# PeterFWS/Structure-PLP-SLAM

Hardware: NVIDIA H100
Metric: frames_per_sec_extract_match_poseopt (higher is better)
Workload: dtype u8/f64

## Files before the change

structure-plp-slam_b200/csrc/orb.cu:

```cuda
#include "common.cuh"
#include <cuda.h>
#include <stdlib.h>
#include "brief_pattern.inc"

namespace plp {

namespace {

constexpr int kMaxLevels = 16;
constexpr int kPatchRadius = 19;
constexpr int kHalfPatch = 15;
constexpr int kCellSize = 64;
constexpr int kOverlap = 6;
constexpr int kCellCap = 1024;

struct LevelInfo {
    int w, h, pitch;
    size_t offset;
    size_t blur_offset;
    int cells_x, cells_y;
    int cell_base;
    int num_cells;
    int budget;
    int slot_base;
// ... 802 lines not shown
    const int g = gx * gy;
    int cur = 0, cur_n = 0, len = 0;
    {
        int *cnts = S.scan;
        for (int i = tid; i < g; i += kQtThreads) cnts[i] = 0;
        __syncthreads();
        for (int i = tid; i < n; i += kQtThreads) {
            const uint32_t c = A.cand[i];
            const unsigned ix = (unsigned)((float)cand_x(c) / dx), iy = (unsigned)((float)cand_y(c) / dy);
            int node = (int)(ix + iy * gx);
            node = min(node, g - 1);
            cls[i] = 0;
            A.owner[0][i] = (unsigned short)node;
            atomicAdd(&cnts[node], 1);
        }
        __syncthreads();
        if (tid == 0) {
            int off = 0, pos = 0;
            for (int i = 0; i < g; ++i) {
                const int c = cnts[i];
                S.newpos[i] = off;
                if (c > 0) {
                    const int ix = i % gx, iy = i / gx;
                    short4 r;
                    r.x = (short)(int)(dx * ix);
                    r.y = (short)(int)(dy * iy);
                    r.z = (short)(int)(dx * (ix + 1));
                    r.w = (short)(int)(dy * (iy + 1));
                    S.rect[0][pos] = r;
                    S.start[0][pos] = (unsigned short)off;
                    S.cnt[0][pos] = (unsigned short)c;
                    S.leaf[0][pos] = (c == 1);
                    S.tot[i] = (unsigned short)pos;
                    ++pos;
                }
                off += c;
            }
            S.misc[0] = pos;
        }
        __syncthreads();
        len = S.misc[0];
        for (int node = 0; node < g; ++node) {
            if (cnts[node] == 0) continue;
            const int per = (n + kQtThreads - 1) / kQtThreads;
            const int i0 = min(n, tid * per), i1 = min(n, i0 + per);
            int c = 0;
            for (int i = i0; i < i1; ++i) c += (A.owner[0][i] == node);
            int tot;
            int run = block_exclusive_scan(c, S.warp_tmp, &tot);
            const int base = S.newpos[node];
            const unsigned short lp = S.tot[node];
            for (int i = i0; i < i1; ++i)
                if (A.owner[0][i] == node) {
                    A.perm[1][base + run] = (unsigned short)i;
                    A.owner[1][base + run] = lp;
                    ++run;
                }
            __syncthreads();
        }
        cur = 1;
    }
    const int budget = LV.budget;
    int pool_len = 0, pool_cur = 0;
    bool filled = false;
    unsigned short *proc_list = S.pool_sorted;

    while (true) {
        const int prev = len;
        for (int p = tid; p < len; p += kQtThreads) S.sel[p] = S.leaf[cur_n][p] ? 0 : 1;
        __syncthreads();
        for (int p = tid; p < len; p += kQtThreads) S.scan[p] = S.sel[p];
        __syncthreads();
        const int num_proc = block_scan_array(S.scan, len, S.warp_tmp);
        for (int p = tid; p < len; p += kQtThreads)
            if (S.sel[p]) proc_list[S.scan[p]] = (unsigned short)p;
        __syncthreads();
        segmented_class_scan(A, cur, n, QtNodes{S.rect[cur_n], S.start[cur_n], S.cnt[cur_n], S.leaf[cur_n]}, S.sel,
                             rank, cls, S.tot, S.carry_tail, S.carry_head);
        len = apply_division(S, A, cur, n, cur_n, len, num_proc, proc_list, rank, cls, &pool_len, pool_cur);
        if (budget <= len || len == prev) {
            filled = true;
            break;
        }
        if (budget < len + pool_len) break;
    }
    while (!filled) {
        const int prev = len;
        const unsigned short *pool = S.pool[pool_cur];
        for (int p = tid; p < len; p += kQtThreads) S.sel[p] = 0;
        __syncthreads();
        for (int k = tid; k < pool_len; k += kQtThreads) S.sel[pool[k]] = 1;
        __syncthreads();
        segmented_class_scan(A, cur, n, QtNodes{S.rect[cur_n], S.start[cur_n], S.cnt[cur_n], S.leaf[cur_n]}, S.sel,
                             rank, cls, S.tot, S.carry_tail, S.carry_head);
        for (int k = tid; k < pool_len; k += kQtThreads) {
            const int ck = S.cnt[cur_n][pool[k]];
            int r = 0;
            for (int j = 0; j < pool_len; ++j) {
                const int cj = S.cnt[cur_n][pool[j]];
                r += (cj > ck) || (cj == ck && j > k);
            }
            proc_list[r] = pool[k];
        }
        __syncthreads();
        for (int k = tid; k < pool_len; k += kQtThreads) {
            const unsigned short *t = S.tot + proc_list[k] * 4;
            S.scan[k] = (t[0] > 0) + (t[1] > 0) + (t[2] > 0) + (t[3] > 0) - 1;
        }
        if (tid == 0) {
            S.misc[1] = pool_len;
            S.misc[2] = 0;
        }
        __syncthreads();
        block_scan_array(S.scan, pool_len, S.warp_tmp);
        for (int k = tid; k < pool_len; k += kQtThreads) {
            const unsigned short *t = S.tot + proc_list[k] * 4;
            const int inc = (t[0] > 0) + (t[1] > 0) + (t[2] > 0) + (t[3] > 0) - 1;
            if (prev + S.scan[k] + inc >= budget) {
                atomicMin(&S.misc[1], k + 1);
                S.misc[2] = 1;
            }
        }
        __syncthreads();
        const int num_proc = S.misc[1];
        const bool reached = S.misc[2] != 0;
        __syncthreads();
        for (int k = num_proc + tid; k < pool_len; k += kQtThreads) S.sel[proc_list[k]] = 0;
        __syncthreads();
        len = apply_division(S, A, cur, n, cur_n, len, num_proc, proc_list, rank, cls, &pool_len, pool_cur ^ 1);
        pool_cur ^= 1;
        if (reached) filled = true;
        if (filled || budget <= len || len == prev) break;
    }

    const int n_out = min(len, LV.slot_cap);
    if (len > LV.slot_cap && tid == 0) P.status[b] = 3;
    for (int p = tid; p < n_out; p += kQtThreads) {
        const int st = S.start[cur_n][p], c = S.cnt[cur_n][p];
        uint32_t best = A.cand[A.perm[cur][st]];
        for (int k = 1; k < c; ++k) {
            const uint32_t v = A.cand[A.perm[cur][st + k]];
            if (cand_score(v) > cand_score(best)) best = v;
        }
        LevelKp kp;
        kp.x = (short)(cand_x(best) + kPatchRadius);
        kp.y = (short)(cand_y(best) + kPatchRadius);
        kp.response = cand_score(best);
        out[p] = kp;
    }
    if (tid == 0) *lvl_cnt = n_out;
}

constexpr int kDescWarps = 4;
constexpr int kBlurDim = 39, kBlurPitch = 44;

__device__ __forceinline__ int reflect101(int p, int len) {
    if (p < 0) p = -p;
    if (p >= len) p = 2 * (len - 1) - p;
    return p;
}

__device__ __forceinline__ float fast_atan2_deg(float y, float x) {
    const float scale = (float)(180.0 / 3.14159265358979323846);
    const float p1 = 0.9997878412794807f * scale, p3 = -0.3258083974640975f * scale,
                p5 = 0.1555786518463281f * scale, p7 = -0.04432655554792128f * scale;
    const float ax = fabsf(x), ay = fabsf(y);
    float a, c, c2;
    if (ax >= ay) {
        c = __fdiv_rn(ay, ax + (float)2.2204460492503131e-16);
        c2 = c * c;
        a = (((p7 * c2 + p5) * c2 + p3) * c2 + p1) * c;
    } else {
        c = __fdiv_rn(ax, ay + (float)2.2204460492503131e-16);
        c2 = c * c;
        a = 90.f - (((p7 * c2 + p5) * c2 + p3) * c2 + p1) * c;
    }
    if (x < 0) a = 180.f - a;
    if (y < 0) a = 360.f - a;
    return a;
}

__device__ __forceinline__ float poly_cos(float v) {
    const float c1 = 0.99940307f, c2 = -0.49558072f, c3 = 0.03679168f;
    const float v2 = v * v;
    return c1 + v2 * (c2 + c3 * v2);
}
__device__ __forceinline__ float util_cos(float v) {
    const float PI = 3.14159265358979f, PI_2 = PI / 2.0f, TWO_PI = 2.0f * PI, INV_TWO_PI = 1.0f / TWO_PI,
                THREE_PI_2 = 3.0f * PI_2;
    v = v - (float)cv_floor((double)(v * INV_TWO_PI)) * TWO_PI;
    v = (0.0f < v) ? v : -v;
    if (v < PI_2) return poly_cos(v);
    if (v < PI) return -poly_cos(PI - v);
    if (v < THREE_PI_2) return -poly_cos(v - PI);
    return poly_cos(TWO_PI - v);
}
__device__ __forceinline__ float util_sin(float v) {
    const float PI_2 = 3.14159265358979f / 2.0f;
    return util_cos(PI_2 - v);
}


__device__ __forceinline__ void blur_row4(const uint32_t *w, uint32_t h[4]) {
    const uint32_t A = w[0], B = w[1], C = w[2];
    const uint32_t kW1 = 0x38302212u, kW2 = 0x00122230u;
    h[0] = __dp4a(__funnelshift_r(A, B, 8), kW1, __dp4a(__funnelshift_r(B, C, 8), kW2, 0u));
    h[1] = __dp4a(__funnelshift_r(A, B, 16), kW1, __dp4a(__funnelshift_r(B, C, 16), kW2, 0u));
    h[2] = __dp4a(__funnelshift_r(A, B, 24), kW1, __dp4a(__funnelshift_r(B, C, 24), kW2, 0u));
    h[3] = __dp4a(B, kW1, __dp4a(C, kW2, 0u));
}
__device__ __forceinline__ void blur_h_pass(const uint8_t *box, uint32_t *h2) {
    const uint32_t *src32 = reinterpret_cast<const uint32_t *>(box);
    for (int i = threadIdx.x; i < (kBoxH / 2) * (kBtW / 4); i += blockDim.x) {
        const int rp = i / (kBtW / 4), j = i % (kBtW / 4);
        const uint32_t *w = src32 + 2 * rp * (kBoxW / 4) + j + (kBoxX - 4) / 4;
        uint32_t e[4], o[4];
        blur_row4(w, e);
        blur_row4(w + kBoxW / 4, o);
        *reinterpret_cast<uint4 *>(h2 + rp * kBtW + 4 * j) =
            make_uint4(__byte_perm(e[0], o[0], 0x5410), __byte_perm(e[1], o[1], 0x5410), __byte_perm(e[2], o[2], 0x5410),
                       __byte_perm(e[3], o[3], 0x5410));
    }
}

constexpr int kBlurThreads = 256;
static_assert((kBtH / 2) * (kBtW / 4) == kBlurThreads, "one vertical-pass job per thread");
__device__ __forceinline__ void blur_v_pass(const uint32_t *h2, uint8_t *dst, int dpitch, int x0, int y0, int W, int H) {
    const int q = threadIdx.x / (kBtW / 4), px = (threadIdx.x % (kBtW / 4)) * 4;
    const int y = y0 + 2 * q;
    if (y >= H || x0 + px >= W) return;
    uint32_t r[4][4];
#pragma unroll
    for (int k = 0; k < 4; ++k) {
        const uint4 v = *reinterpret_cast<const uint4 *>(h2 + (q + k) * kBtW + px);
        r[k][0] = v.x;
        r[k][1] = v.y;
        r[k][2] = v.z;
        r[k][3] = v.w;
    }
    auto row = [&](uint32_t k0, uint32_t k1, uint32_t k2, uint32_t k3) -> uint32_t {
        uint32_t a[4];
#pragma unroll
        for (int c = 0; c < 4; ++c)
            a[c] = __dp2a_lo(r[0][c], k0, __dp2a_lo(r[1][c], k1, __dp2a_lo(r[2][c], k2, __dp2a_lo(r[3][c], k3, 32768u))));
        return __byte_perm(__byte_perm(a[0], a[1], 0x0062), __byte_perm(a[2], a[3], 0x0062), 0x5410);
    };
    uint8_t *d = dst + (size_t)y * dpitch + x0 + px;
    *reinterpret_cast<uint32_t *>(d) = row(0x2212u, 0x3830u, 0x2230u, 0x0012u);
    if (y + 1 < H) *reinterpret_cast<uint32_t *>(d + dpitch) = row(0x1200u, 0x3022u, 0x3038u, 0x1222u);
}

__global__ void __launch_bounds__(kBlurThreads) blur_tiles_kernel(OrbDev P) {
    __shared__ __align__(16) uint8_t s_src[kBoxH * kBoxW];
    __shared__ __align__(16) uint32_t s_h2[(kBoxH / 2) * kBtW];
    const int b = blockIdx.y, tid = threadIdx.x;
    const BlurTile t = P.blur_tiles[blockIdx.x];
    const int l = t.level, W = P.lv[l].w, H = P.lv[l].h;
    const uint8_t *img = level_ptr(P, b, l);
    const int pitch = level_pitch(P, l);
    constexpr int kCols = kBtW + 8;
    for (int i = tid; i < kBoxH * kCols; i += kBlurThreads) {
        const int py = i / kCols, px = i - py * kCols;
        const int gy = reflect101(min(t.y0 - 3 + py, H + 2), H);
        const int gx = reflect101(min(max(t.x0 - 4 + px, -3), W + 2), W);
        s_src[py * kBoxW + kBoxX - 4 + px] = img[(size_t)gy * pitch + gx];
    }
    __syncthreads();
    blur_h_pass(s_src, s_h2);
    __syncthreads();
    blur_v_pass(s_h2, P.blur + (size_t)b * P.blur_frame_bytes + P.lv[l].blur_offset, P.lv[l].pitch, t.x0, t.y0, W, H);
}

__device__ void blur_reflect_box(uint8_t *box, int bx0, int by0, int W, int H) {
    for (int i = threadIdx.x; i < kBoxH * 6; i += blockDim.x) {
        const int py = i / 6, k = i - py * 6;
        const int gx = k < 3 ? k - 3 : W + (k - 3), gy = by0 + py;
        const int px = gx - bx0;
        if (gy < 0 || gy >= H || px < 0 || px >= kBoxW) continue;
        box[py * kBoxW + px] = box[py * kBoxW + (reflect101(gx, W) - bx0)];
    }
    __syncthreads();
    for (int i = threadIdx.x; i < 6 * kBoxW; i += blockDim.x) {
        const int k = i / kBoxW, px = i - k * kBoxW;
        const int gy = k < 3 ? k - 3 : H + (k - 3);
        const int py = gy - by0;
        if (py < 0 || py >= kBoxH) continue;
        box[py * kBoxW + px] = box[(reflect101(gy, H) - by0) * kBoxW + px];
    }
    __syncthreads();
}

constexpr int kBlurRun = 4;
template <bool kMapsInGlobal>
__global__ void __launch_bounds__(kBlurThreads) blur_tiles_tma_kernel(const __grid_constant__ BlurMaps M, const CUtensorMap *gmaps,
                                                                      OrbDev P, int run) {
    __shared__ __align__(128) uint8_t s_src[2][kBoxStage];
    __shared__ __align__(16) uint32_t s_h2[(kBoxH / 2) * kBtW];
    __shared__ __align__(8) unsigned long long s_bar[2];
    const int b = blockIdx.y, tid = threadIdx.x;
    const int first = blockIdx.x * run, n = min(run, P.num_blur_tiles - first);
    if (tid == 0) {
        mbar_init(smem_u32(&s_bar[0]));
        mbar_init(smem_u32(&s_bar[1]));
        asm volatile("fence.mbarrier_init.release.cluster;" ::: "memory");
    }
    __syncthreads();
    auto issue = [&](int i) {
        const BlurTile t = P.blur_tiles[first + i];
        const uint32_t bar = smem_u32(&s_bar[i & 1]);
        mbar_expect_tx(bar, kBoxH * kBoxW);
        tma_box_load(smem_u32(s_src[i & 1]), level_map<kMapsInGlobal>(M, gmaps, t.level), t.x0 - kBoxX, t.y0 - 3, b, bar);
    };
    if (tid == 0) issue(0);
    for (int i = 0; i < n; ++i) {
        __syncthreads();
        if (tid == 0 && i + 1 < n) {
            asm volatile("fence.proxy.async.shared::cta;" ::: "memory");
            issue(i + 1);
        }
        const BlurTile t = P.blur_tiles[first + i];
        const int l = t.level, W = P.lv[l].w, H = P.lv[l].h;
        const int bx0 = t.x0 - kBoxX, by0 = t.y0 - 3;
        uint8_t *box = s_src[i & 1];
        if (!mbar_wait(smem_u32(&s_bar[i & 1]), (i >> 1) & 1)) P.status[b] = 3;
        if (t.x0 < 3 || by0 < 0 || t.x0 + kBtW + 3 > W || by0 + kBoxH > H) blur_reflect_box(box, bx0, by0, W, H);
        blur_h_pass(box, s_h2);
        __syncthreads();
        blur_v_pass(s_h2, P.blur + (size_t)b * P.blur_frame_bytes + P.lv[l].blur_offset, P.lv[l].pitch, t.x0, t.y0, W, H);
    }
}

__global__ void __launch_bounds__(kDescWarps * 32) describe_kernel(OrbDev P, plp_keypoint *__restrict__ kp_out,
                                                                    uint8_t *__restrict__ desc_out,
                                                                    int32_t *__restrict__ n_out) {
    __shared__ __align__(16) uint8_t s_win[kDescWarps][kBlurDim * kBlurPitch];
    const int b = blockIdx.y, warp = threadIdx.x >> 5, lane = threadIdx.x & 31;
    __shared__ int s_cum[kMaxLevels + 1];
    __shared__ const uint8_t *s_img[kMaxLevels], *s_blur[kMaxLevels];
    __shared__ int s_pitch[kMaxLevels], s_bpitch[kMaxLevels], s_slot[kMaxLevels];
    __shared__ float s_scale[kMaxLevels], s_size[kMaxLevels];
    if (threadIdx.x == 0) {
        const int *lvl_cnt = P.lvl_cnt + (size_t)b * P.num_levels;
        int acc = 0;
        for (int l = 0; l < P.num_levels; ++l) {
            s_cum[l] = acc;
            acc += lvl_cnt[l];
        }
        for (int l = P.num_levels; l <= kMaxLevels; ++l) s_cum[l] = acc;
    }
    if (threadIdx.x < P.num_levels) {
        const int l = threadIdx.x;
        s_img[l] = level_ptr(P, b, l);
        s_pitch[l] = level_pitch(P, l);
        s_blur[l] = P.blur + (size_t)b * P.blur_frame_bytes + P.lv[l].blur_offset;
        s_bpitch[l] = P.lv[l].pitch;
        s_slot[l] = P.lv[l].slot_base;
        s_scale[l] = P.lv[l].scale_factor;
        s_size[l] = P.lv[l].size;
    }
    __syncthreads();
    const int total = min(s_cum[kMaxLevels], P.out_cap);
    if (blockIdx.x == 0 && threadIdx.x == 0) n_out[b] = total;
    const LevelKp *frame_kp = P.lvl_kp + (size_t)b * P.total_slots;
    for (int out_pos = blockIdx.x * kDescWarps + warp; out_pos < total; out_pos += gridDim.x * kDescWarps) {
    int l = 0;
    while (out_pos >= s_cum[l + 1]) ++l;
    const LevelKp kp = frame_kp[s_slot[l] + out_pos - s_cum[l]];
    const uint8_t *img = s_img[l];
    const int pitch = s_pitch[l];
    const int cx = kp.x, cy = kp.y;

    int m10 = 0, m01 = 0;
    {
        constexpr int kUmax[16] = {15, 15, 15, 15, 14, 14, 14, 13, 13, 12, 11, 10, 9, 8, 6, 3};
        const int u = lane - kHalfPatch;
        const int au = u < 0 ? -u : u;
        const uint8_t *c0 = img + (size_t)cy * pitch + cx + u;
#pragma unroll
        for (int v = -kHalfPatch; v <= kHalfPatch; ++v) {
            const int d = kUmax[v < 0 ? -v : v];
            if (lane < 31 && au <= d) {
                const int val = __ldg(c0 + v * pitch);
                m10 += u * val;
                m01 += v * val;
            }
        }
#pragma unroll
        for (int o = 16; o > 0; o >>= 1) {
            m10 += __shfl_xor_sync(0xffffffffu, m10, o);
            m01 += __shfl_xor_sync(0xffffffffu, m01, o);
        }
    }
    const float angle = fast_atan2_deg((float)m01, (float)m10);

    const float ang_rad = (float)((double)angle * 3.14159265358979323846 / 180.0);
    const float ca = util_cos(ang_rad), sa = util_sin(ang_rad);
    const int bpitch = s_bpitch[l];
    const int wx0 = cx - 19, woff = wx0 & 3, nwords = (woff + kBlurDim + 3) >> 2;
    const uint8_t *bsrc = s_blur[l] + (size_t)(cy - 19) * bpitch + (wx0 - woff);
    uint8_t *win = s_win[warp];
    __syncwarp();
    {
        const int half = lane >> 4, j = lane & 15;
        if (j < nwords) {
#pragma unroll 5
            for (int r = half; r < kBlurDim; r += 2)
                *reinterpret_cast<uint32_t *>(win + r * kBlurPitch + 4 * j) =
                    __ldg(reinterpret_cast<const uint32_t *>(bsrc + (size_t)r * bpitch) + j);
        }
    }
    __syncwarp();
    const uint8_t *center = win + 19 * kBlurPitch + 19 + woff;
    int val = 0;
    const uint2 px1 = __ldg(reinterpret_cast<const uint2 *>(kBriefX1) + lane), py1 = __ldg(reinterpret_cast<const uint2 *>(kBriefY1) + lane);
    const uint2 px2 = __ldg(reinterpret_cast<const uint2 *>(kBriefX2) + lane), py2 = __ldg(reinterpret_cast<const uint2 *>(kBriefY2) + lane);
#pragma unroll
    for (int bit = 0; bit < 8; ++bit) {
        const int sh = (bit & 3) * 8;
        const float x1 = (float)(signed char)(((bit < 4 ? px1.x : px1.y) >> sh) & 0xff);
        const float y1 = (float)(signed char)(((bit < 4 ? py1.x : py1.y) >> sh) & 0xff);
        const float x2 = (float)(signed char)(((bit < 4 ? px2.x : px2.y) >> sh) & 0xff);
        const float y2 = (float)(signed char)(((bit < 4 ? py2.x : py2.y) >> sh) & 0xff);
        const int r1 = __float2int_rn(x1 * sa + y1 * ca), c1 = __float2int_rn(x1 * ca - y1 * sa);
        const int r2 = __float2int_rn(x2 * sa + y2 * ca), c2 = __float2int_rn(x2 * ca - y2 * sa);
        val |= (center[r1 * kBlurPitch + c1] < center[r2 * kBlurPitch + c2]) << bit;
    }
    desc_out[((size_t)b * P.out_cap + out_pos) * 32 + lane] = (uint8_t)val;
    if (lane == 0) {
        plp_keypoint o;
        const float s = s_scale[l];
        o.x = l == 0 ? (float)cx : (float)cx * s;
        o.y = l == 0 ? (float)cy : (float)cy * s;
        o.size = s_size[l];
        o.angle = angle;
        o.response = (float)kp.response;
        o.octave = l;
        o.class_id = -1;
        kp_out[(size_t)b * P.out_cap + out_pos] = o;
    }
    }
}

}

}

using namespace plp;

struct plp_orb {
    plp_ctx *ctx = nullptr;
    plp_orb_params params;
    int rows = 0, cols = 0, max_batch = 0;
    OrbDev dev;
    std::vector<float> scale_factors, inv_scale_factors, level_sigma_sq, inv_level_sigma_sq;
    std::vector<uint32_t> num_keypts_per_level;
    std::vector<CellDesc> cells;
    short4 *d_xtab[kMaxLevels] = {nullptr};
    short4 *d_ytab[kMaxLevels] = {nullptr};
    CellDesc *d_cells = nullptr;
    uint8_t *d_pyr = nullptr;
    uint8_t *d_blur = nullptr;
    BlurTile *d_blur_tiles = nullptr;
    std::vector<BlurTile> blur_tiles;
    uint8_t *d_img = nullptr;
    uint8_t *d_mask = nullptr;
    uint32_t *d_cell_buf = nullptr;
    int *d_cell_cnt = nullptr;
    LevelKp *d_lvl_kp = nullptr;
    int *d_lvl_cnt = nullptr;
    uint8_t *d_qt_scratch = nullptr;
    int *d_status = nullptr;
    plp_keypoint *d_kp = nullptr;
    uint8_t *d_desc = nullptr;
    int32_t *d_n = nullptr;
    size_t qt_smem = 0;
    bool qt_small = false;
    BlurMaps maps;
    bool maps_ok = false;
    bool no_tma = false;
    bool maps_global = false;
    CUtensorMap *d_maps = nullptr;
    bool d_maps_dirty = true;
    const uint8_t *map0_img = nullptr;
    size_t map0_step = 0;
    int map0_batch = 0;
    int last_batch = 0;
    const uint8_t *last_img0 = nullptr;
    size_t last_step = 0;
};

typedef CUresult (*EncodeTiledFn)(CUtensorMap *, CUtensorMapDataType, cuuint32_t, void *, const cuuint64_t *, const cuuint64_t *,
                                  const cuuint32_t *, const cuuint32_t *, CUtensorMapInterleave, CUtensorMapSwizzle,
                                  CUtensorMapL2promotion, CUtensorMapFloatOOBfill);
static EncodeTiledFn tensor_map_encoder() {
    static EncodeTiledFn fn = []() -> EncodeTiledFn {
        void *p = nullptr;
        cudaDriverEntryPointQueryResult q;
        if (cudaGetDriverEntryPoint("cuTensorMapEncodeTiled", &p, cudaEnableDefault, &q) != cudaSuccess ||
            q != cudaDriverEntryPointSuccess)
            return nullptr;
        return (EncodeTiledFn)p;
    }();
    return fn;
}
static bool encode_level_map(CUtensorMap *m, const uint8_t *base, int w, int h, int frames, size_t pitch, size_t frame_stride) {
    EncodeTiledFn enc = tensor_map_encoder();
    if (!enc || ((uintptr_t)base & 15) || (pitch & 15) || (frame_stride & 15) || w < 1 || h < 1 || frames < 1) return false;
    const cuuint64_t dims[3] = {(cuuint64_t)w, (cuuint64_t)h, (cuuint64_t)frames};
    const cuuint64_t strides[2] = {(cuuint64_t)pitch, (cuuint64_t)frame_stride};
    const cuuint32_t box[3] = {(cuuint32_t)kBoxW, (cuuint32_t)kBoxH, 1u}, estr[3] = {1u, 1u, 1u};
    return enc(m, CU_TENSOR_MAP_DATA_TYPE_UINT8, 3, (void *)base, dims, strides, box, estr, CU_TENSOR_MAP_INTERLEAVE_NONE,
               CU_TENSOR_MAP_SWIZZLE_NONE, CU_TENSOR_MAP_L2_PROMOTION_L2_128B, CU_TENSOR_MAP_FLOAT_OOB_FILL_NONE) == CUDA_SUCCESS;
}


static void build_resize_tables(int sw, int sh, int dw, int dh, std::vector<short4> &xt, std::vector<short4> &yt) {
    const double inv_scale_x = (double)dw / sw, inv_scale_y = (double)dh / sh;
    const double scale_x = 1. / inv_scale_x, scale_y = 1. / inv_scale_y;
    xt.resize(dw);
    yt.resize(dh);
    for (int dx = 0; dx < dw; ++dx) {
        float fx = (float)((dx + 0.5) * scale_x - 0.5);
        int sx = cv_floor(fx);
        fx -= sx;
        if (sx < 0) {
            fx = 0;
            sx = 0;
        }
        if (sx >= sw - 1) {
            fx = 0;
            sx = sw - 1;
        }
        short4 t;
        t.x = (short)sx;
        t.y = (short)std::min(sx + 1, sw - 1);
        t.z = (short)lrintf((1.f - fx) * 2048);
        t.w = (short)lrintf(fx * 2048);
        xt[dx] = t;
    }
    for (int dy = 0; dy < dh; ++dy) {
        float fy = (float)((dy + 0.5) * scale_y - 0.5);
        int sy = cv_floor(fy);
        fy -= sy;
        short4 t;
        t.x = (short)std::min(std::max(sy, 0), sh - 1);
        t.y = (short)std::min(std::max(sy + 1, 0), sh - 1);
        t.z = (short)lrintf((1.f - fy) * 2048);
        t.w = (short)lrintf(fy * 2048);
        yt[dy] = t;
    }
}

extern "C" {

void plp_orb_destroy(plp_orb *o) {
    if (!o) return;
    cudaSetDevice(o->ctx->device);
    cudaStreamSynchronize(o->ctx->stream);
    for (int l = 0; l < kMaxLevels; ++l) {
        if (o->d_xtab[l]) cudaFree(o->d_xtab[l]);
        if (o->d_ytab[l]) cudaFree(o->d_ytab[l]);
    }
    void *ptrs[] = {o->d_blur, o->d_blur_tiles, o->d_cells, o->d_pyr, o->d_img, o->d_mask, o->d_cell_buf, o->d_cell_cnt, o->d_lvl_kp,
                    o->d_lvl_cnt, o->d_qt_scratch, o->d_status, o->d_kp, o->d_desc, o->d_n, o->d_maps};
    for (void *p : ptrs)
        if (p) cudaFree(p);
    delete o;
}

plp_status plp_orb_create(plp_ctx *ctx, const plp_orb_params *params, int rows, int cols, int max_batch,
                          plp_orb **out) {
    PLP_REQUIRE(ctx && params && out, "null pointer");
    *out = nullptr;
    PLP_REQUIRE(rows > 0 && cols > 0 && max_batch > 0, "image size / batch");
    PLP_REQUIRE(params->num_levels >= 1 && params->num_levels <= kMaxLevels, "num_levels in [1,16]");
    PLP_REQUIRE(params->scale_factor > 1.0f || params->num_levels == 1, "scale_factor > 1");
    PLP_REQUIRE(cols <= 2047 + 2 * kPatchRadius && rows <= 1023 + 2 * kPatchRadius,
                "image larger than 2085 x 1061 (packed candidate coordinates)");
    PLP_REQUIRE(params->ini_fast_thr < 255 && params->min_fast_thr >= 1 && params->min_fast_thr <= params->ini_fast_thr,
                "FAST thresholds: 1 <= min <= ini < 255");
    PLP_CUDA_TRY(cudaSetDevice(ctx->device));
    plp_orb *o = new plp_orb();
    {
        const char *nt = getenv("PLP_BLUR_NO_TMA");
        o->no_tma = nt && nt[0] == '1';
        const char *mg = getenv("PLP_TMA_MAPS");
        o->maps_global = mg && mg[0] == 'g';
    }
    o->ctx = ctx;
    o->params = *params;
    o->rows = rows;
    o->cols = cols;
// ... 127 lines not shown
    D.num_cells = cell_base;
    D.total_slots = slot_base;
    D.out_cap = slot_base;
    D.pyr_frame_bytes = pyr_bytes ? pyr_bytes : 256;
    D.blur_frame_bytes = blur_bytes ? blur_bytes : 256;
    D.num_blur_tiles = (int)o->blur_tiles.size();
    const size_t B = (size_t)max_batch;
#define ORB_ALLOC(ptr, bytes)                                              \
    do {                                                                   \
        cudaError_t e_ = cudaMalloc((void **)&(ptr), (bytes) ? (bytes) : 256); \
        if (e_ != cudaSuccess) {                                           \
            set_error("orb: cudaMalloc(%zu) failed: %s", (size_t)(bytes), cudaGetErrorString(e_)); \
            plp_orb_destroy(o);                                            \
            return PLP_ERR_CUDA;                                           \
        }                                                                  \
    } while (0)
    for (unsigned l = 1; l < L; ++l) {
        std::vector<short4> xt, yt;
        build_resize_tables(D.lv[l - 1].w, D.lv[l - 1].h, D.lv[l].w, D.lv[l].h, xt, yt);
        ORB_ALLOC(o->d_xtab[l], xt.size() * sizeof(short4));
        ORB_ALLOC(o->d_ytab[l], yt.size() * sizeof(short4));
        cudaMemcpy(o->d_xtab[l], xt.data(), xt.size() * sizeof(short4), cudaMemcpyHostToDevice);
        cudaMemcpy(o->d_ytab[l], yt.data(), yt.size() * sizeof(short4), cudaMemcpyHostToDevice);
    }
    ORB_ALLOC(o->d_cells, o->cells.size() * sizeof(CellDesc));
    if (!o->cells.empty())
        cudaMemcpy(o->d_cells, o->cells.data(), o->cells.size() * sizeof(CellDesc), cudaMemcpyHostToDevice);
    ORB_ALLOC(o->d_pyr, B * D.pyr_frame_bytes);
    ORB_ALLOC(o->d_blur, B * D.blur_frame_bytes);
    ORB_ALLOC(o->d_blur_tiles, o->blur_tiles.size() * sizeof(BlurTile));
    if (!o->blur_tiles.empty())
        cudaMemcpy(o->d_blur_tiles, o->blur_tiles.data(), o->blur_tiles.size() * sizeof(BlurTile), cudaMemcpyHostToDevice);
    ORB_ALLOC(o->d_img, B * (size_t)rows * cols);
    ORB_ALLOC(o->d_mask, (size_t)rows * cols);
    ORB_ALLOC(o->d_cell_buf, B * (size_t)D.num_cells * kCellCap * sizeof(uint32_t));
    ORB_ALLOC(o->d_cell_cnt, B * (size_t)D.num_cells * sizeof(int));
    ORB_ALLOC(o->d_lvl_kp, B * (size_t)D.total_slots * sizeof(LevelKp));
    ORB_ALLOC(o->d_lvl_cnt, B * L * sizeof(int));
    D.qt_scratch_per_job = (size_t)65536 * (4 + 2 * 5 + 1) + 256;
    ORB_ALLOC(o->d_qt_scratch, B * L * D.qt_scratch_per_job);
    ORB_ALLOC(o->d_status, B * sizeof(int));
    ORB_ALLOC(o->d_maps, sizeof(BlurMaps));
    ORB_ALLOC(o->d_kp, B * (size_t)D.out_cap * sizeof(plp_keypoint));
    ORB_ALLOC(o->d_desc, B * (size_t)D.out_cap * 32);
    ORB_ALLOC(o->d_n, B * sizeof(int32_t));
#undef ORB_ALLOC
    D.pyr = o->d_pyr;
    D.blur = o->d_blur;
    D.blur_tiles = o->d_blur_tiles;
    D.cells = o->d_cells;
    D.cell_buf = o->d_cell_buf;
    D.cell_cnt = o->d_cell_cnt;
    D.lvl_kp = o->d_lvl_kp;
    D.lvl_cnt = o->d_lvl_cnt;
    D.qt_scratch = o->d_qt_scratch;
    D.status = o->d_status;
    o->maps_ok = true;
    memset(&o->maps, 0, sizeof(o->maps));
    for (unsigned l = 1; l < L && o->maps_ok; ++l)
        o->maps_ok = encode_level_map(&o->maps.m[l], o->d_pyr + D.lv[l].offset, D.lv[l].w, D.lv[l].h, max_batch, D.lv[l].pitch,
                                      D.pyr_frame_bytes);
    o->qt_small = qt_max_slots <= kNodeCapSmall && !getenv("PLP_QT_LARGE");
    plp_status so;
    if (o->qt_small) {
        o->qt_smem = ((sizeof(QtSharedT<kNodeCapSmall>) + 15) & ~(size_t)15) + (size_t)kCandCapSmall * (4 + 2 * 5 + 1) + 64;
        so = ensure_smem_optin((const void *)quadtree_kernel<kNodeCapSmall, kCandCapSmall, 2>, o->qt_smem, "quadtree_kernel<small>");
    } else {
        o->qt_smem = ((sizeof(QtSharedT<kNodeCap>) + 15) & ~(size_t)15) + (size_t)kCandCapLarge * (4 + 2 * 5 + 1) + 64;
        so = ensure_smem_optin((const void *)quadtree_kernel<kNodeCap, kCandCapLarge, 1>, o->qt_smem, "quadtree_kernel<large>");
    }
    if (so != PLP_OK) {
        plp_orb_destroy(o);
        return so;
    }
    *out = o;
    return PLP_OK;
}

int plp_orb_capacity(const plp_orb *o) { return o ? o->dev.out_cap : 0; }

plp_status plp_orb_get_tables(const plp_orb *o, float *sf, float *isf, float *ls, float *ils, uint32_t *nk) {
    PLP_REQUIRE(o, "orb");
    for (int l = 0; l < o->dev.num_levels; ++l) {
        if (sf) sf[l] = o->scale_factors[l];
        if (isf) isf[l] = o->inv_scale_factors[l];
        if (ls) ls[l] = o->level_sigma_sq[l];
        if (ils) ils[l] = o->inv_level_sigma_sq[l];
        if (nk) nk[l] = o->num_keypts_per_level[l];
    }
    return PLP_OK;
}

static plp_status orb_run(plp_orb *o, const uint8_t *d_imgs, int batch, size_t step, const uint8_t *d_mask,
                          size_t mask_step, plp_keypoint *d_kp, uint8_t *d_desc, int32_t *d_n, int32_t *d_status) {
    plp_ctx *ctx = o->ctx;
    OrbDev D = o->dev;
    D.img0 = d_imgs;
    D.img0_step = step;
    D.img0_frame_stride = step * (size_t)o->rows;
    D.mask = d_mask;
    D.mask_step = mask_step;
    D.status = d_status ? d_status : o->d_status;
    o->last_batch = batch;
    o->last_img0 = d_imgs;
    o->last_step = step;
    PLP_CUDA_TRY(cudaMemsetAsync(D.status, 0, (size_t)batch * sizeof(int), ctx->stream));
    for (int l = 1; l < D.num_levels; ++l) {
        const int quads = ((D.lv[l].w + 3) >> 2) * ((D.lv[l].h + kResizeRows - 1) / kResizeRows);
        if (quads <= 0) continue;
        dim3 grid(div_up(quads, 256), batch);
        PLP_LAUNCH(ctx, pyr_resize_kernel, grid, 256, 0, D, l, o->d_xtab[l], o->d_ytab[l]);
    }
    bool tma = o->maps_ok && !o->no_tma;
    if (tma && (o->map0_img != d_imgs || o->map0_step != step || o->map0_batch != batch)) {
        tma = encode_level_map(&o->maps.m[0], d_imgs, D.lv[0].w, D.lv[0].h, batch, step, D.img0_frame_stride);
        o->map0_img = tma ? d_imgs : nullptr;
        o->d_maps_dirty = true;
        o->map0_step = step;
        o->map0_batch = batch;
    }
    if (tma && o->maps_global && o->d_maps_dirty) {
        PLP_CUDA_TRY(cudaMemcpyAsync(o->d_maps, &o->maps, sizeof(BlurMaps), cudaMemcpyHostToDevice, ctx->stream));
        o->d_maps_dirty = false;
    }
    if (D.num_cells > 0) {
        dim3 grid(D.num_cells, batch), grid_run(div_up(D.num_cells, kFastRun), batch);
        if (tma && o->maps_global)
            PLP_LAUNCH(ctx, fast_cells_tma_kernel<true>, grid_run, 256, 0, o->maps, o->d_maps, D, kFastRun);
        else if (tma)
            PLP_LAUNCH(ctx, fast_cells_tma_kernel<false>, grid_run, 256, 0, o->maps, (const CUtensorMap *)nullptr, D, kFastRun);
        else
            PLP_LAUNCH(ctx, fast_cells_kernel_v2, grid, 256, 0, D);
    }
    if (D.num_blur_tiles > 0) {
        dim3 grid(D.num_blur_tiles, batch), grid_run(div_up(D.num_blur_tiles, kBlurRun), batch);
        if (tma && o->maps_global)
            PLP_LAUNCH(ctx, blur_tiles_tma_kernel<true>, grid_run, kBlurThreads, 0, o->maps, o->d_maps, D, kBlurRun);
        else if (tma)
            PLP_LAUNCH(ctx, blur_tiles_tma_kernel<false>, grid_run, kBlurThreads, 0, o->maps, (const CUtensorMap *)nullptr, D, kBlurRun);
        else
            PLP_LAUNCH(ctx, blur_tiles_kernel, grid, kBlurThreads, 0, D);
    }
    {
        dim3 grid(D.num_levels, batch);
        if (ctx->timing) plp::timing_begin(ctx, o->qt_small ? "quadtree_kernel<1024>" : "quadtree_kernel<2048>");
        if (o->qt_small)
            quadtree_kernel<kNodeCapSmall, kCandCapSmall, 2><<<grid, kQtThreads, o->qt_smem, ctx->stream>>>(D);
        else
            quadtree_kernel<kNodeCap, kCandCapLarge, 1><<<grid, kQtThreads, o->qt_smem, ctx->stream>>>(D);
        if (ctx->timing) plp::timing_end(ctx);
        ctx->launches++;
    }
    {
        const int kp_est = std::max(256, (int)(3 * o->params.max_num_keypts / 2));
        dim3 grid(div_up(std::min(D.total_slots, kp_est), kDescWarps), batch);
        PLP_LAUNCH(ctx, describe_kernel, grid, kDescWarps * 32, 0, D, d_kp, d_desc, d_n);
    }
    PLP_CHECK_LAUNCH();
    return PLP_OK;
}

plp_status plp_orb_extract_batch_dev(plp_orb *o, const uint8_t *d_imgs, int batch, size_t step, plp_keypoint *d_kp,
                                     uint8_t *d_desc, int32_t *d_n, int32_t *d_status) {
    PLP_REQUIRE(o && d_imgs && d_kp && d_desc && d_n, "null pointer");
    PLP_REQUIRE(batch >= 1 && batch <= o->max_batch, "batch exceeds the handle's max_batch");
    PLP_REQUIRE(step >= (size_t)o->cols, "step < cols");
    PLP_CUDA_TRY(cudaSetDevice(o->ctx->device));
    return orb_run(o, d_imgs, batch, step, nullptr, 0, d_kp, d_desc, d_n, d_status);
}

static plp_status orb_extract_host(plp_orb *o, const uint8_t *imgs, int batch, size_t step, const uint8_t *mask,
                                   size_t mask_step, plp_keypoint *kp_out, uint8_t *desc_out, int32_t *n_out) {
    plp_ctx *ctx = o->ctx;
    PLP_CUDA_TRY(cudaSetDevice(ctx->device));
    const size_t rows = o->rows, cols = o->cols;
    PLP_CUDA_TRY(cudaMemcpy2DAsync(o->d_img, cols, imgs, step, cols, rows * (size_t)batch, cudaMemcpyHostToDevice,
                                   ctx->stream));
    const uint8_t *d_mask = nullptr;
    if (mask) {
        PLP_CUDA_TRY(cudaMemcpy2DAsync(o->d_mask, cols, mask, mask_step, cols, rows, cudaMemcpyHostToDevice, ctx->stream));
        d_mask = o->d_mask;
    }
    PLP_TRY(orb_run(o, o->d_img, batch, cols, d_mask, cols, o->d_kp, o->d_desc, o->d_n, nullptr));
    const size_t cap = o->dev.out_cap;
    PLP_CUDA_TRY(cudaMemcpyAsync(n_out, o->d_n, (size_t)batch * 4, cudaMemcpyDeviceToHost, ctx->stream));
    PLP_CUDA_TRY(cudaMemcpyAsync(kp_out, o->d_kp, (size_t)batch * cap * sizeof(plp_keypoint), cudaMemcpyDeviceToHost,
                                 ctx->stream));
    PLP_CUDA_TRY(cudaMemcpyAsync(desc_out, o->d_desc, (size_t)batch * cap * 32, cudaMemcpyDeviceToHost, ctx->stream));
    std::vector<int> status(batch);
    PLP_CUDA_TRY(cudaMemcpyAsync(status.data(), o->d_status, (size_t)batch * 4, cudaMemcpyDeviceToHost, ctx->stream));
    PLP_CUDA_TRY(cudaStreamSynchronize(ctx->stream));
    for (int b = 0; b < batch; ++b)
        if (status[b] != 0) {
            set_error("orb: capacity overflow in frame %d (code %d)", b, status[b]);
            return PLP_ERR_CAPACITY;
        }
    return PLP_OK;
}

plp_status plp_orb_extract(plp_orb *o, const uint8_t *img, int rows, int cols, size_t step, const uint8_t *mask,
                           size_t mask_step, plp_keypoint *kp_out, uint8_t *desc_out, int *n_out) {
    PLP_REQUIRE(o && n_out, "null pointer");
    *n_out = 0;
    if (!img || rows == 0 || cols == 0) return PLP_OK;
    PLP_REQUIRE(rows == o->rows && cols == o->cols, "image size differs from the handle's");
    PLP_REQUIRE(kp_out && desc_out, "null output");
    PLP_REQUIRE(step >= (size_t)cols && (!mask || mask_step >= (size_t)cols), "step < cols");
    int32_t n = 0;
    PLP_TRY(orb_extract_host(o, img, 1, step, mask, mask_step, kp_out, desc_out, &n));
    *n_out = n;
    return PLP_OK;
}

plp_status plp_orb_extract_batch(plp_orb *o, const uint8_t *imgs, int batch, size_t step, plp_keypoint *kp_out,
                                 uint8_t *desc_out, int32_t *n_out) {
    PLP_REQUIRE(o && imgs && kp_out && desc_out && n_out, "null pointer");
    PLP_REQUIRE(batch >= 1 && batch <= o->max_batch, "batch exceeds the handle's max_batch");
    PLP_REQUIRE(step >= (size_t)o->cols, "step < cols");
    return orb_extract_host(o, imgs, batch, step, nullptr, 0, kp_out, desc_out, n_out);
}

plp_status plp_orb_get_pyramid(const plp_orb *o, int b, int level, plp_image_view *out) {
    PLP_REQUIRE(o && out, "null pointer");
    PLP_REQUIRE(b >= 0 && b < o->last_batch && level >= 0 && level < o->dev.num_levels, "index");
    const LevelInfo &V = o->dev.lv[level];
    out->rows = V.h;
    out->cols = V.w;
    if (level == 0) {
        out->data = o->last_img0 + (size_t)b * o->last_step * o->rows;
        out->step = o->last_step;
    } else {
        out->data = o->d_pyr + (size_t)b * o->dev.pyr_frame_bytes + V.offset;
        out->step = V.pitch;
    }
    return PLP_OK;
}

plp_status plp_orb_debug_blurred(plp_orb *o, int b, int level, uint8_t *out) {
    PLP_REQUIRE(o && out, "null pointer");
    PLP_REQUIRE(b >= 0 && b < o->last_batch && level >= 0 && level < o->dev.num_levels, "index");
    plp_ctx *ctx = o->ctx;
    PLP_CUDA_TRY(cudaSetDevice(ctx->device));
    const LevelInfo &V = o->dev.lv[level];
    PLP_CUDA_TRY(cudaStreamSynchronize(ctx->stream));
    PLP_CUDA_TRY(cudaMemcpy2D(out, V.w, o->d_blur + (size_t)b * o->dev.blur_frame_bytes + V.blur_offset, V.pitch, V.w, V.h,
                              cudaMemcpyDeviceToHost));
    return PLP_OK;
}

plp_status plp_orb_debug_candidates(plp_orb *o, int b, int level, plp_keypoint *out, int cap, int *n_out) {
    PLP_REQUIRE(o && out && n_out, "null pointer");
    PLP_REQUIRE(b >= 0 && b < o->last_batch && level >= 0 && level < o->dev.num_levels, "index");
    plp_ctx *ctx = o->ctx;
    PLP_CUDA_TRY(cudaSetDevice(ctx->device));
    const LevelInfo &V = o->dev.lv[level];
    std::vector<int> cnt(V.num_cells);
    std::vector<uint32_t> buf((size_t)V.num_cells * kCellCap);
    PLP_CUDA_TRY(cudaStreamSynchronize(ctx->stream));
    if (V.num_cells) {
        PLP_CUDA_TRY(cudaMemcpy(cnt.data(), o->d_cell_cnt + (size_t)b * o->dev.num_cells + V.cell_base,
                                cnt.size() * 4, cudaMemcpyDeviceToHost));
        PLP_CUDA_TRY(cudaMemcpy(buf.data(), o->d_cell_buf + ((size_t)b * o->dev.num_cells + V.cell_base) * kCellCap,
                                buf.size() * 4, cudaMemcpyDeviceToHost));
    }
    int n = 0;
    for (int c = 0; c < V.num_cells; ++c)
        for (int k = 0; k < cnt[c]; ++k) {
            if (n < cap) {
                const uint32_t v = buf[(size_t)c * kCellCap + k];
                plp_keypoint kp;
                kp.x = (float)(v & 0x7ff);
                kp.y = (float)((v >> 11) & 0x3ff);
                kp.size = 7.f;
                kp.angle = -1.f;
                kp.response = (float)(v >> 21);
                kp.octave = 0;
                kp.class_id = -1;
                out[n] = kp;
            }
            ++n;
        }
    *n_out = n;
    return PLP_OK;
}

}
```

Baseline: 80570.

## Pipeline describe kernel with cp.async double-buffered patch staging and dp4a moments

Each warp now handles a run of eight keypoints and prefetches the next keypoint's intensity disc and blurred window into a two-slot shared-memory ring with cp.async while it computes the current one. The orientation moments use dp4a against per-lane weight masks in place of per-pixel scalar loads, and the BRIEF pattern coordinates are decoded once per thread. Level prefix sums move to a warp shuffle scan, and the grid is resized for the per-warp runs. This is meant to hide global-load latency and cut instruction count, at the cost of more shared memory, more registers, and fewer warps when keypoints are few.

Measured after the change: 87960, median of 6. 9.2% higher.

```diff
diff --git a/structure-plp-slam_b200/csrc/orb.cu b/structure-plp-slam_b200/csrc/orb.cu
--- a/structure-plp-slam_b200/csrc/orb.cu
+++ b/structure-plp-slam_b200/csrc/orb.cu
@@ -978,7 +978,14 @@
 }
 
 constexpr int kDescWarps = 4;
-constexpr int kBlurDim = 39, kBlurPitch = 44;
+constexpr int kDescRun = 8;
+constexpr int kDescMinBlocks = 5;
+constexpr int kDiscRows = 2 * kHalfPatch + 1, kDiscPitch = 48;
+constexpr int kWinHalf = 18, kWinRows = 2 * kWinHalf + 1, kWinPitch = 64;
+constexpr int kDiscBytes = kDiscRows * kDiscPitch;
+constexpr int kDescStage = kDiscBytes + kWinRows * kWinPitch;
+static_assert(kDiscBytes % 16 == 0 && kDescStage % 16 == 0, "16-byte copies into every row of the ring");
+static_assert(15 + kDiscRows <= kDiscPitch && 15 + kWinRows <= kWinPitch, "the aligned supersets fit the rows");
 
 __device__ __forceinline__ int reflect101(int p, int len) {
     if (p < 0) p = -p;
@@ -1156,114 +1163,189 @@
     }
 }
 
-__global__ void __launch_bounds__(kDescWarps * 32) describe_kernel(OrbDev P, plp_keypoint *__restrict__ kp_out,
+__device__ __forceinline__ void cp_async16(void *dst, const void *src) {
+    asm volatile("cp.async.ca.shared.global [%0], [%1], 16;" ::"r"(smem_u32(dst)), "l"(src) : "memory");
+}
+__device__ __forceinline__ void cp_async_commit() { asm volatile("cp.async.commit_group;" ::: "memory"); }
+__device__ __forceinline__ void cp_async_wait_prev() { asm volatile("cp.async.wait_group 1;" ::: "memory"); }
+
+__device__ __forceinline__ int dp4a_us(uint32_t a, uint32_t b, int c) {
+    int d;
+    asm("dp4a.u32.s32 %0, %1, %2, %3;" : "=r"(d) : "r"(a), "r"(b), "r"(c));
+    return d;
+}
+
+template <int J>
+__device__ __forceinline__ void disc_row_sums(const uint32_t (&r)[12], int sh, const uint32_t (&wu)[8],
+                                              const uint32_t (&wm)[8], int &su, int &si) {
+#pragma unroll
+    for (int k = 0; k < 8; ++k) {
+        const uint32_t w = __funnelshift_r(r[J + k], r[J + k + 1], sh);
+        su = dp4a_us(w, wu[k], su);
+        si = dp4a_us(w, wm[k], si);
+    }
+}
+
+__global__ void __launch_bounds__(kDescWarps * 32, kDescMinBlocks) describe_kernel(OrbDev P, plp_keypoint *__restrict__ kp_out,
                                                                     uint8_t *__restrict__ desc_out,
                                                                     int32_t *__restrict__ n_out) {
-    __shared__ __align__(16) uint8_t s_win[kDescWarps][kBlurDim * kBlurPitch];
-    const int b = blockIdx.y, warp = threadIdx.x >> 5, lane = threadIdx.x & 31;
+    __shared__ __align__(16) uint8_t s_ring[kDescWarps][2][kDescStage];
     __shared__ int s_cum[kMaxLevels + 1];
     __shared__ const uint8_t *s_img[kMaxLevels], *s_blur[kMaxLevels];
     __shared__ int s_pitch[kMaxLevels], s_bpitch[kMaxLevels], s_slot[kMaxLevels];
     __shared__ float s_scale[kMaxLevels], s_size[kMaxLevels];
-    if (threadIdx.x == 0) {
-        const int *lvl_cnt = P.lvl_cnt + (size_t)b * P.num_levels;
-        int acc = 0;
-        for (int l = 0; l < P.num_levels; ++l) {
-            s_cum[l] = acc;
-            acc += lvl_cnt[l];
-        }
-        for (int l = P.num_levels; l <= kMaxLevels; ++l) s_cum[l] = acc;
-    }
-    if (threadIdx.x < P.num_levels) {
-        const int l = threadIdx.x;
-        s_img[l] = level_ptr(P, b, l);
-        s_pitch[l] = level_pitch(P, l);
-        s_blur[l] = P.blur + (size_t)b * P.blur_frame_bytes + P.lv[l].blur_offset;
-        s_bpitch[l] = P.lv[l].pitch;
-        s_slot[l] = P.lv[l].slot_base;
-        s_scale[l] = P.lv[l].scale_factor;
-        s_size[l] = P.lv[l].size;
+    const int b = blockIdx.y, warp = threadIdx.x >> 5, lane = threadIdx.x & 31;
+    if (warp == 0) {
+        const int l = lane;
+        int c = l < P.num_levels ? P.lvl_cnt[(size_t)b * P.num_levels + l] : 0;
+#pragma unroll
+        for (int o = 1; o < 32; o <<= 1) {
+            const int t = __shfl_up_sync(0xffffffffu, c, o);
+            if (lane >= o) c += t;
+        }
+        if (l == 0) s_cum[0] = 0;
+        if (l < kMaxLevels) s_cum[l + 1] = c;
+        if (l < P.num_levels) {
+            s_img[l] = level_ptr(P, b, l);
+            s_pitch[l] = level_pitch(P, l);
+            s_blur[l] = P.blur + (size_t)b * P.blur_frame_bytes + P.lv[l].blur_offset;
+            s_bpitch[l] = P.lv[l].pitch;
+            s_slot[l] = P.lv[l].slot_base;
+            s_scale[l] = P.lv[l].scale_factor;
+            s_size[l] = P.lv[l].size;
+        }
+    }
+    const bool vec0 = ((reinterpret_cast<uintptr_t>(P.img0) | P.img0_step | P.img0_frame_stride) & 15) == 0;
+    uint32_t wu[8], wm[8];
+    {
+        const int dv = lane - kHalfPatch, umax = lane < kDiscRows ? P.u_max[dv < 0 ? -dv : dv] : -1;
+#pragma unroll
+        for (int k = 0; k < 8; ++k) {
+            wu[k] = wm[k] = 0;
+#pragma unroll
+            for (int c = 0; c < 4; ++c) {
+                const int u = 4 * k + c - kHalfPatch;
+                if (u <= kHalfPatch && (u < 0 ? -u : u) <= umax) {
+                    wu[k] |= (uint32_t)(u & 0xff) << (8 * c);
+                    wm[k] |= 1u << (8 * c);
+                }
+            }
+        }
+    }
+    float x1[8], y1[8], x2[8], y2[8];
+    {
+        const uint2 px1 = __ldg(reinterpret_cast<const uint2 *>(kBriefX1) + lane), py1 = __ldg(reinterpret_cast<const uint2 *>(kBriefY1) + lane);
+        const uint2 px2 = __ldg(reinterpret_cast<const uint2 *>(kBriefX2) + lane), py2 = __ldg(reinterpret_cast<const uint2 *>(kBriefY2) + lane);
+#pragma unroll
+        for (int bit = 0; bit < 8; ++bit) {
+            const int sh = (bit & 3) * 8;
+            x1[bit] = (float)(signed char)(((bit < 4 ? px1.x : px1.y) >> sh) & 0xff);
+            y1[bit] = (float)(signed char)(((bit < 4 ? py1.x : py1.y) >> sh) & 0xff);
+            x2[bit] = (float)(signed char)(((bit < 4 ? px2.x : px2.y) >> sh) & 0xff);
+            y2[bit] = (float)(signed char)(((bit < 4 ? py2.x : py2.y) >> sh) & 0xff);
+        }
     }
     __syncthreads();
     const int total = min(s_cum[kMaxLevels], P.out_cap);
     if (blockIdx.x == 0 && threadIdx.x == 0) n_out[b] = total;
     const LevelKp *frame_kp = P.lvl_kp + (size_t)b * P.total_slots;
-    for (int out_pos = blockIdx.x * kDescWarps + warp; out_pos < total; out_pos += gridDim.x * kDescWarps) {
-    int l = 0;
-    while (out_pos >= s_cum[l + 1]) ++l;
-    const LevelKp kp = frame_kp[s_slot[l] + out_pos - s_cum[l]];
-    const uint8_t *img = s_img[l];
-    const int pitch = s_pitch[l];
-    const int cx = kp.x, cy = kp.y;
-
-    int m10 = 0, m01 = 0;
-    {
-        constexpr int kUmax[16] = {15, 15, 15, 15, 14, 14, 14, 13, 13, 12, 11, 10, 9, 8, 6, 3};
-        const int u = lane - kHalfPatch;
-        const int au = u < 0 ? -u : u;
-        const uint8_t *c0 = img + (size_t)cy * pitch + cx + u;
-#pragma unroll
-        for (int v = -kHalfPatch; v <= kHalfPatch; ++v) {
-            const int d = kUmax[v < 0 ? -v : v];
-            if (lane < 31 && au <= d) {
-                const int val = __ldg(c0 + v * pitch);
-                m10 += u * val;
-                m01 += v * val;
+    uint8_t(*ring)[kDescStage] = s_ring[warp];
+    for (int p0 = (blockIdx.x * kDescWarps + warp) * kDescRun; p0 < total; p0 += gridDim.x * kDescWarps * kDescRun) {
+        const int n = min(kDescRun, total - p0);
+        int ml = 0, mx = 0, my = 0, mresp = 0;
+        if (lane < n) {
+            const int pos = p0 + lane;
+            while (pos >= s_cum[ml + 1]) ++ml;
+            const LevelKp kp = frame_kp[s_slot[ml] + pos - s_cum[ml]];
+            mx = kp.x;
+            my = kp.y;
+            mresp = kp.response;
+        }
+        auto stage = [&](int i) {
+            const int cx = __shfl_sync(0xffffffffu, mx, i), cy = __shfl_sync(0xffffffffu, my, i),
+                      l = __shfl_sync(0xffffffffu, ml, i);
+            uint8_t *disc = ring[i & 1], *win = disc + kDiscBytes;
+            const int xw = cx - kWinHalf, ow = xw & 15, nw = (ow + kWinRows + 15) >> 4, bpitch = s_bpitch[l];
+            const uint8_t *bsrc = s_blur[l] + (size_t)(cy - kWinHalf) * bpitch + (xw - ow);
+#pragma unroll
+            for (int t = lane; t < kWinRows * 4; t += 32) {
+                const int r = t >> 2, c = t & 3;
+                if (c < nw) cp_async16(win + r * kWinPitch + 16 * c, bsrc + (size_t)r * bpitch + 16 * c);
             }
-        }
-#pragma unroll
-        for (int o = 16; o > 0; o >>= 1) {
-            m10 += __shfl_xor_sync(0xffffffffu, m10, o);
-            m01 += __shfl_xor_sync(0xffffffffu, m01, o);
-        }
-    }
-    const float angle = fast_atan2_deg((float)m01, (float)m10);
-
-    const float ang_rad = (float)((double)angle * 3.14159265358979323846 / 180.0);
-    const float ca = util_cos(ang_rad), sa = util_sin(ang_rad);
-    const int bpitch = s_bpitch[l];
-    const int wx0 = cx - 19, woff = wx0 & 3, nwords = (woff + kBlurDim + 3) >> 2;
-    const uint8_t *bsrc = s_blur[l] + (size_t)(cy - 19) * bpitch + (wx0 - woff);
-    uint8_t *win = s_win[warp];
-    __syncwarp();
-    {
-        const int half = lane >> 4, j = lane & 15;
-        if (j < nwords) {
-#pragma unroll 5
-            for (int r = half; r < kBlurDim; r += 2)
-                *reinterpret_cast<uint32_t *>(win + r * kBlurPitch + 4 * j) =
-                    __ldg(reinterpret_cast<const uint32_t *>(bsrc + (size_t)r * bpitch) + j);
-        }
-    }
-    __syncwarp();
-    const uint8_t *center = win + 19 * kBlurPitch + 19 + woff;
-    int val = 0;
-    const uint2 px1 = __ldg(reinterpret_cast<const uint2 *>(kBriefX1) + lane), py1 = __ldg(reinterpret_cast<const uint2 *>(kBriefY1) + lane);
-    const uint2 px2 = __ldg(reinterpret_cast<const uint2 *>(kBriefX2) + lane), py2 = __ldg(reinterpret_cast<const uint2 *>(kBriefY2) + lane);
-#pragma unroll
-    for (int bit = 0; bit < 8; ++bit) {
-        const int sh = (bit & 3) * 8;
-        const float x1 = (float)(signed char)(((bit < 4 ? px1.x : px1.y) >> sh) & 0xff);
-        const float y1 = (float)(signed char)(((bit < 4 ? py1.x : py1.y) >> sh) & 0xff);
-        const float x2 = (float)(signed char)(((bit < 4 ? px2.x : px2.y) >> sh) & 0xff);
-        const float y2 = (float)(signed char)(((bit < 4 ? py2.x : py2.y) >> sh) & 0xff);
-        const int r1 = __float2int_rn(x1 * sa + y1 * ca), c1 = __float2int_rn(x1 * ca - y1 * sa);
-        const int r2 = __float2int_rn(x2 * sa + y2 * ca), c2 = __float2int_rn(x2 * ca - y2 * sa);
-        val |= (center[r1 * kBlurPitch + c1] < center[r2 * kBlurPitch + c2]) << bit;
-    }
-    desc_out[((size_t)b * P.out_cap + out_pos) * 32 + lane] = (uint8_t)val;
-    if (lane == 0) {
-        plp_keypoint o;
-        const float s = s_scale[l];
-        o.x = l == 0 ? (float)cx : (float)cx * s;
-        o.y = l == 0 ? (float)cy : (float)cy * s;
-        o.size = s_size[l];
-        o.angle = angle;
-        o.response = (float)kp.response;
-        o.octave = l;
-        o.class_id = -1;
-        kp_out[(size_t)b * P.out_cap + out_pos] = o;
-    }
+            const int xd = cx - kHalfPatch, od = xd & 15, pitch = s_pitch[l];
+            const uint8_t *dsrc = s_img[l] + (size_t)(cy - kHalfPatch) * pitch;
+            if (l > 0 || vec0) {
+                const int nd = (od + kDiscRows + 15) >> 4;
+                dsrc += xd - od;
+#pragma unroll
+                for (int t = lane; t < kDiscRows * 3; t += 32) {
+                    const int r = t / 3, c = t - 3 * r;
+                    if (c < nd) cp_async16(disc + r * kDiscPitch + 16 * c, dsrc + (size_t)r * pitch + 16 * c);
+                }
+            } else if (lane < kDiscRows) {
+#pragma unroll 8
+                for (int r = 0; r < kDiscRows; ++r)
+                    disc[r * kDiscPitch + od + lane] = __ldg(dsrc + (size_t)r * pitch + xd + lane);
+            }
+        };
+        stage(0);
+        cp_async_commit();
+        float my_angle = 0.f;
+        for (int i = 0; i < n; ++i) {
+            if (i + 1 < n) stage(i + 1);
+            cp_async_commit();
+            cp_async_wait_prev();
+            __syncwarp();
+            const int cx = __shfl_sync(0xffffffffu, mx, i);
+            const uint8_t *disc = ring[i & 1], *win = disc + kDiscBytes;
+
+            int su = 0, si = 0;
+            {
+                const uint4 *row = reinterpret_cast<const uint4 *>(disc + min(lane, kDiscRows - 1) * kDiscPitch);
+                const uint4 q0 = row[0], q1 = row[1], q2 = row[2];
+                const uint32_t r[12] = {q0.x, q0.y, q0.z, q0.w, q1.x, q1.y, q1.z, q1.w, q2.x, q2.y, q2.z, q2.w};
+                const int od = (cx - kHalfPatch) & 15, sh = 8 * (od & 3);
+                switch (od >> 2) {
+                    case 0: disc_row_sums<0>(r, sh, wu, wm, su, si); break;
+                    case 1: disc_row_sums<1>(r, sh, wu, wm, su, si); break;
+                    case 2: disc_row_sums<2>(r, sh, wu, wm, su, si); break;
+                    default: disc_row_sums<3>(r, sh, wu, wm, su, si); break;
+                }
+            }
+            int m10 = su, m01 = (lane - kHalfPatch) * si;
+#pragma unroll
+            for (int o = 16; o > 0; o >>= 1) {
+                m10 += __shfl_xor_sync(0xffffffffu, m10, o);
+                m01 += __shfl_xor_sync(0xffffffffu, m01, o);
+            }
+            const float angle = fast_atan2_deg((float)m01, (float)m10);
+
+            const float ang_rad = (float)((double)angle * 3.14159265358979323846 / 180.0);
+            const float ca = util_cos(ang_rad), sa = util_sin(ang_rad);
+            const uint8_t *center = win + kWinHalf * kWinPitch + kWinHalf + ((cx - kWinHalf) & 15);
+            int val = 0;
+#pragma unroll
+            for (int bit = 0; bit < 8; ++bit) {
+                const int r1 = __float2int_rn(x1[bit] * sa + y1[bit] * ca), c1 = __float2int_rn(x1[bit] * ca - y1[bit] * sa);
+                const int r2 = __float2int_rn(x2[bit] * sa + y2[bit] * ca), c2 = __float2int_rn(x2[bit] * ca - y2[bit] * sa);
+                val |= (center[r1 * kWinPitch + c1] < center[r2 * kWinPitch + c2]) << bit;
+            }
+            desc_out[((size_t)b * P.out_cap + p0 + i) * 32 + lane] = (uint8_t)val;
+            if (lane == i) my_angle = angle;
+            __syncwarp();
+        }
+        if (lane < n) {
+            plp_keypoint o;
+            const float s = s_scale[ml];
+            o.x = ml == 0 ? (float)mx : (float)mx * s;
+            o.y = ml == 0 ? (float)my : (float)my * s;
+            o.size = s_size[ml];
+            o.angle = my_angle;
+            o.response = (float)mresp;
+            o.octave = ml;
+            o.class_id = -1;
+            kp_out[(size_t)b * P.out_cap + p0 + lane] = o;
+        }
     }
 }
 
@@ -1697,8 +1779,8 @@
         ctx->launches++;
     }
     {
-        const int kp_est = std::max(256, (int)(3 * o->params.max_num_keypts / 2));
-        dim3 grid(div_up(std::min(D.total_slots, kp_est), kDescWarps), batch);
+        const int kp_est = std::max(256, (int)o->params.max_num_keypts);
+        dim3 grid(div_up(std::min(D.total_slots, kp_est), kDescWarps * kDescRun), batch);
         PLP_LAUNCH(ctx, describe_kernel, grid, kDescWarps * 32, 0, D, d_kp, d_desc, d_n);
     }
     PLP_CHECK_LAUNCH();
```
